# CleConor/rivulus

Measured on AMD Instinct MI355X. Metric: rows/sec filter+project, 1e9-row Int64, 10% selectivity, higher is better.
Workload: dtype int64

## Files before the change

rivulus_amd/csrc/core.hip:

```cpp
#include "launch.hpp"

using namespace rvh;
using namespace rvl;

namespace {
thread_local std::string g_last_error_text;
}
std::string &rvh::last_error() { return g_last_error_text; }

namespace rvl {

size_t elem_bytes(rv_dtype t, uint64_t n) {
    switch (t) {
        case RV_INT64:
        case RV_FLOAT64: return static_cast<size_t>(n) * 8;
        case RV_BOOLEAN: return static_cast<size_t>((n + 63) / 64) * 8;
        default: return 0;
    }
}
size_t bitmap_words_bytes(uint64_t n) { return static_cast<size_t>((n + 63) / 64) * 8; }

DevBufRef pool_alloc(rv_ctx *ctx, size_t bytes) {
    auto b = std::make_shared<DevBuf>();
    size_t got = 0;
// ... 73 lines not shown
    for (size_t i = 0; i < ctx->ctrl_free.size(); ++i)
        if (ctx->ctrl_free[i].bytes >= need) {
            c = ctx->ctrl_free[i];
            ctx->ctrl_free.erase(ctx->ctrl_free.begin() + static_cast<long>(i));
            break;
        }
    if (!c.dev) {
        if (!ctx->ctrl_free.empty()) {
            c = ctx->ctrl_free.back();
            ctx->ctrl_free.pop_back();
            RV_HIP(hipStreamSynchronize(ctx->stream));
            RV_HIP(hipFree(c.dev));
            c.dev = nullptr;
        } else {
            RV_HIP(hipHostMalloc(&c.host, kCtrlBytes, hipHostMallocDefault));
            RV_HIP(hipEventCreateWithFlags(&c.ev, hipEventDisableTiming));
        }
        c.bytes = std::max(need + need / 2, static_cast<size_t>(1) << 16);
        RV_HIP(hipMalloc(&c.dev, c.bytes));
    }
    RV_HIP(hipMemsetAsync(c.dev, 0, (zeroed + 15) & ~size_t(15), ctx->stream));
    c.clean = 0;
    c.dirty = zeroed;
    return c;
}
void release_launch_ctrl(rv_ctx *ctx, const rv_ctx::LaunchCtrl &c) { ctx->ctrl_free.push_back(c); }
int block_to_zero(rv_ctx *ctx, const rv_ctx::LaunchCtrl &like) {
    constexpr size_t kMost = size_t(64) << 20;
    for (size_t i = 0; i < ctx->ctrl_free.size(); ++i)
        if (ctx->ctrl_free[i].clean == 0 && ctx->ctrl_free[i].dirty > 0 && ctx->ctrl_free[i].dirty <= kMost) return static_cast<int>(i);
    bool any_clean = false;
    for (auto &f : ctx->ctrl_free) any_clean = any_clean || f.clean > 0;
    if (any_clean || ctx->ctrl_free.size() >= 3 || like.bytes > kMost) return -1;
    rv_ctx::LaunchCtrl c;
    if (hipHostMalloc(&c.host, kCtrlBytes, hipHostMallocDefault) != hipSuccess || hipEventCreateWithFlags(&c.ev, hipEventDisableTiming) != hipSuccess ||
        hipMalloc(&c.dev, like.bytes) != hipSuccess) {
        (void)hipGetLastError();
        if (c.host) (void)hipHostFree(c.host);
        if (c.ev) (void)hipEventDestroy(c.ev);
        return -1;
    }
    c.bytes = like.bytes;
    c.dirty = like.dirty;
    ctx->ctrl_free.push_back(c);
    return static_cast<int>(ctx->ctrl_free.size()) - 1;
}

rvk::DevCol dev_view(const rv_dcolumn *c) {
    rvk::DevCol d{};
    d.values = c->values ? c->values->ptr : nullptr;
// ... 86 lines not shown
    return count;
}

rv_status rv_ctx_create(int device, rv_ctx **out) {
    return guarded([&] {
        require(out != nullptr, RV_ERR_INVALID_ARG, "rv_ctx_create: out is NULL");
        int count = 0;
        hipError_t e = hipGetDeviceCount(&count);
        if (e != hipSuccess || count == 0) {
            (void)hipGetLastError();
            throw Error(RV_ERR_DEVICE, "no HIP device available: the MI355X backend has no CPU fallback");
        }
        require(device >= 0 && device < count, RV_ERR_INVALID_ARG, fmt("device %d out of range (%d present)", device, count));
        auto ctx = std::make_unique<rv_ctx>();
        ctx->device = device;
        RV_HIP(hipSetDevice(device));
        RV_HIP(hipGetDeviceProperties(&ctx->props, device));
        require(std::string(ctx->props.gcnArchName).rfind("gfx950", 0) == 0, RV_ERR_DEVICE,
                fmt("device %d is %s; this library carries gfx950 (MI355X) code objects only", device, ctx->props.gcnArchName));
        RV_HIP(hipStreamCreateWithFlags(&ctx->stream, hipStreamNonBlocking));
        RV_HIP(hipEventCreate(&ctx->ev0));
        RV_HIP(hipEventCreate(&ctx->ev1));
        RV_HIP(hipEventCreate(&ctx->evk0));
        RV_HIP(hipEventCreate(&ctx->evk1));
        RV_HIP(hipHostMalloc(&ctx->h_ctrl, kCtrlBytes, hipHostMallocDefault));
        RV_HIP(hipMalloc(&ctx->d_stripes, kStripeBytes));
        RV_HIP(hipMemset(ctx->d_stripes, 0, kStripeBytes));
        ctx->pool = std::make_shared<Pool>(device);
        if (const char *env = getenv("RV_OPTIONS")) {
            std::string all(env);
// ... 91 lines not shown
        else if (k == "stamp") ctx->opt_stamp = value;
        else if (k == "debug") ctx->opt_debug = value;
        else if (k == "depth") ctx->opt_depth = value;
        else if (k == "roomy") ctx->opt_roomy = value;
        else if (k == "direct") ctx->opt_direct = value;
        else if (k == "direct_r") ctx->opt_direct_r = value;
        else if (k == "sample") ctx->opt_sample = value;
        else if (k == "skew") ctx->opt_skew = value;
        else if (k == "segments") ctx->opt_segments = value;
        else if (k == "str_tiles_from") ctx->opt_str_tiles_from = value;
        else if (k == "groups_by_ranges") ctx->opt_groups_by_ranges = value;
        else if (k == "bool_cap") ctx->opt_bool_cap = value;
        else if (k == "speculative_batches") ctx->opt_speculative_batches = value;
        else if (k == "direct_waves") ctx->opt_direct_waves = value;
        else if (k == "spin_limit") ctx->opt_spin_limit = value;
        else if (k == "agg_grid") ctx->opt_agg_grid = value;
        else if (k == "bools_in_pass") ctx->opt_bools_in_pass = value;
        else if (k == "narrow_codes") {
            require(value >= -1 && value <= 2, RV_ERR_INVALID_ARG, "narrow_codes: 0 (auto), -1 (never), 1 (at the first whole scan, never packed) or 2 (at the first whole scan, packed where the rule allows)");
            ctx->opt_narrow_codes = value;
        }
        else if (k == "inject_failure") ctx->opt_inject_failure = value;
        else if (k == "csv_slow_cap") {
            require(value >= 0 && value < (int64_t(1) << 31), RV_ERR_INVALID_ARG, "csv_slow_cap must be in [0, 2^31)");
            ctx->opt_csv_slow_cap = value;
        }
        else if (k == "join_hash_bits") {
            require(value >= 0 && value < 64, RV_ERR_INVALID_ARG, "join_hash_bits must be in [0, 64)");
            ctx->opt_join_hash_bits = value;
        }
// ... 68 lines not shown
        else if (k == "csv_slow_cells") *value = static_cast<int64_t>(ctx->csv_slow_cells);
        else if (k == "csv_slow_reparses") *value = static_cast<int64_t>(ctx->csv_slow_reparses);
        else if (k == "inject_failure") *value = ctx->opt_inject_failure;
        else if (k == "join_hash_bits") *value = ctx->opt_join_hash_bits;
        else if (k == "string_hash_bits") *value = ctx->opt_string_hash_bits;
        else if (k == "agg_hash_bits") *value = ctx->opt_agg_hash_bits;
        else if (k == "agg_max_groups") *value = ctx->opt_agg_max_groups;
        else if (k == "sort_engine") *value = ctx->opt_sort_engine;
        else if (k == "sort_last_passes") *value = static_cast<int64_t>(ctx->sort_last_passes);
        else if (k == "top_k_select_from_rows") *value = ctx->opt_top_k_select_from_rows;
        else if (k == "top_k_refine_divisor") *value = ctx->opt_top_k_refine_divisor;
        else if (k == "top_k_last_passes") *value = static_cast<int64_t>(ctx->top_k_last_passes);
        else if (k == "top_k_last_candidates") *value = static_cast<int64_t>(ctx->top_k_last_candidates);
        else if (k == "out_sizing") *value = ctx->opt_out_sizing;
        else if (k == "overflow_reruns") *value = static_cast<int64_t>(ctx->overflow_reruns);
        else if (k == "batch_counts_in_pass") *value = static_cast<int64_t>(ctx->batch_counts_in_pass);
        else if (k == "fused_rows_scanned") *value = static_cast<int64_t>(ctx->fused_rows_scanned);
        else if (k == "last_redo_ppm") *value = static_cast<int64_t>(ctx->last_redo_fraction * 1e6);
        else if (k == "last_selectivity_ppm") *value = ctx->last_selectivity < 0 ? -1 : static_cast<int64_t>(ctx->last_selectivity * 1e6);
        else throw Error(RV_ERR_INVALID_ARG, "unknown option '" + k + "'");
    });
}

rv_status rv_ctx_kernel_stats(rv_ctx *ctx, double *total_ms, uint64_t *launches, int reset) {
    return guarded([&] {
        require(ctx != nullptr, RV_ERR_INVALID_ARG, "ctx is NULL");
        if (total_ms) *total_ms = ctx->kernel_ms;
        if (launches) *launches = ctx->kernel_launches;
        if (reset) {
            ctx->kernel_ms = 0.0;
// ... 29 lines not shown
```

rivulus_amd/csrc/fused_kernel.hpp:

```cpp
#pragma once

#include "lookback.hpp"
#include "narrow_sides.hpp"
#include "scan_frontend.hpp"
#include "tile_addr.hpp"

namespace rvk {

struct FusedParams {
    ScanInputs in;
    BitStream xs[kMaxBitStreams];
    uint64_t *out_values[kMaxValueCols];
    uint64_t *out_validity[kMaxValueCols];
    unsigned long long *out_valid_pop;
    uint64_t *out_selection;
    uint64_t *state;
    uint32_t *ticket;
    unsigned long long *out_count;
    uint32_t *err;
    uint32_t *overflow;
    uint64_t out_capacity;
    uint32_t *redo_count;
    unsigned long long *redo;
    unsigned long long *stamps;
    uint32_t ntiles;
    uint32_t cap_rows;
    int32_t nxs;
    int32_t debug;
    int32_t depth;
    uint32_t spin_limit;
    uint32_t out_bias;
    uint32_t *wave_counts;
    rv_u32x4 *zero_ptr;
    uint64_t zero_n16;
    unsigned long long *batch_counts;
    uint64_t nbatch_counts;
    uint64_t *wave_offsets;
    NarrowView narrow;
};

static_assert(kMaxTerms >= 4, "term slots 1 to 3 carry a one-term launch's code interval and tile constants");
__host__ __device__ inline void put_tile_walk(ScanInputs &in, const rvtile::TileWalk &w) {
    in.terms[2].lit = static_cast<int64_t>(w.view_byte0);
    in.terms[2].packed = w.tile_bytes;
    in.terms[2].pad = w.wave_bytes;
    in.terms[3].lit = static_cast<int64_t>(w.bytes);
    in.terms[3].packed = w.first_ragged_tile;
    in.terms[3].pad = w.ragged_rows;
}
__host__ __device__ inline rvtile::TileWalk get_tile_walk(const ScanInputs &in) {
    rvtile::TileWalk w{};
    w.view_byte0 = static_cast<uint64_t>(in.terms[2].lit);
    w.tile_bytes = in.terms[2].packed;
    w.wave_bytes = in.terms[2].pad;
// ... 859 lines not shown
            atomicAdd(&d[1], st_scatter);
            atomicAdd(&d[2], st_look);
            atomicAdd(&d[3], st_waitB);
            atomicAdd(&d[4], st_flush);
            atomicAdd(&d[5], st_tiles);
            if (wave == 1) {
                atomicAdd(&d[6], st_wait);
                atomicAdd(&d[7], st_stage);
            }
        }
    }

    if (__syncthreads_or(n_redo != 0)) {
        if (lane == 0 && n_redo) atomicAdd(s_redo, n_redo);
        __syncthreads();
        if (threadIdx.x == 0) atomicAdd(p.redo_count, *s_redo);
    }

    if constexpr (kValidity || kXs) {
        __syncthreads();
        const uint32_t *s_pop = reinterpret_cast<const uint32_t *>(smem + 24);
        if (threadIdx.x < kMaxValueCols + kMaxBitStreams && s_pop[threadIdx.x])
            atomicAdd(&p.out_valid_pop[threadIdx.x], static_cast<unsigned long long>(s_pop[threadIdx.x]));
    }
}

#undef RV_TILE_PARAM
#undef RV_TILE_WRITES

constexpr int kRedoWaves = 4;
template <int NCOLS, int RR>
// ... 125 lines not shown
```

rivulus_amd/csrc/fused_launch.hip:

```cpp
#include "fused_rule.hpp"
#include "launch.hpp"
#include "narrow_sides.hpp"
#include "narrow_term.hpp"
#include "tile_addr.hpp"

#include <cmath>

using namespace rvh;
using namespace rvl;

namespace rvk {
const FusedEntry *fused_entries(size_t *n) {
    static const std::vector<FusedEntry> all = [] {
        std::vector<FusedEntry> v;
        for (auto *source : {fused_entries_lean1, fused_entries_valid1, fused_entries_multi, fused_entries_bool, fused_entries_full, fused_entries_expr,
                             fused_entries_roomy, fused_entries_narrow}) {
            size_t k = 0;
            const FusedEntry *t = source(&k);
            v.insert(v.end(), t, t + k);
        }
        return v;
    }();
    *n = all.size();
    return all.data();
// ... 108 lines not shown
        mix(ex->negate_result ? 3 : 2);
        for (size_t t = 0; t < ex->negate.size(); ++t) mix(static_cast<uint64_t>(ex->negate[t]) | (static_cast<uint64_t>(ex->group_end[t]) << 8));
    }
    return signature;
}

static void launch_redo(rv_ctx *ctx, FusedLaunch &L) {
    const int rr = L.nvals ? rvk::redo_rows_per_lane(L.nvals, L.range_rows) : 4;
    const rvk::RedoFn redo = rvk::redo_kernel(L.nvals, rr);
    require(redo != nullptr && L.nranges > 0, RV_ERR_INTERNAL, "no redo kernel variant");
    const size_t redo_lds = rvk::kLdsHeader + static_cast<size_t>(rvk::kRedoWaves) * (std::max(L.nvals, 1) + rvk::kMaxBitStreams) * 64 * rr;
    const uint64_t want = (L.nranges + rvk::kRedoWaves - 1) / rvk::kRedoWaves;
    const uint32_t rgrid = static_cast<uint32_t>(std::min<uint64_t>(want, static_cast<uint64_t>(ctx->props.multiProcessorCount) * 8));
    hipLaunchKernelGGL(redo, dim3(rgrid), dim3(rvk::kRedoWaves * 64), redo_lds, ctx->stream, L.p, L.range_rows, L.nranges);
    RV_HIP(hipGetLastError());
}

struct Bound {
    const rv_dcolumn *const *cols;
    rvk::ScanInputs *in;
    std::vector<int> value_slot, bool_slot;
    std::vector<char> never_null;
    int nvals = 0, nbools = 0, npred = 0;

    int add_value(const rv_dcolumn *col) {
        require(nvals < rvk::kMaxValueCols, RV_ERR_UNSUPPORTED, "too many 8-byte columns for one pass");
        in->cols[nvals] = dev_view(col);
        return nvals++;
    }
    int value_of(uint32_t c) {
// ... 350 lines not shown
}

static void launch_pass(rv_ctx *ctx, FusedLaunch &L, const LaunchChoice &c, int nvals, rv_dcolumn **sel_out, BatchReq *req, RangeOffsets *ranges,
                        double seen) {
    rvk::FusedParams &p = L.p;
    if (c.make_selection) make_selection(ctx, L, sel_out);
    p.ntiles = c.ntiles;
    p.cap_rows = c.cap;
    p.depth = static_cast<int32_t>(c.stages) - 1;

    L.range_rows = 64u * static_cast<uint32_t>(c.r);
    L.nranges = c.direct ? 0 : static_cast<uint64_t>(p.ntiles) * c.waves;
    L.ctrl = acquire_launch_ctrl(ctx, p.ntiles, L.nranges);
    Ctrl *ctrl = static_cast<Ctrl *>(L.ctrl.dev);
    p.state = reinterpret_cast<uint64_t *>(static_cast<unsigned char *>(L.ctrl.dev) + kCtrlBytes);
    p.ticket = &ctrl->ticket;
    p.err = &ctrl->err;
    p.out_count = &ctrl->out_count;
    p.out_valid_pop = ctrl->valid_pop;
    p.stamps = ctrl->stamps;
    p.debug = static_cast<int32_t>(ctx->opt_debug);
    p.spin_limit = ctx->opt_spin_limit > 0 ? static_cast<uint32_t>(ctx->opt_spin_limit) : rvk::kSpinLimit;
    p.redo_count = &ctrl->redo_count;
    p.redo = L.nranges ? reinterpret_cast<unsigned long long *>(static_cast<unsigned char *>(L.ctrl.dev) + kCtrlBytes + static_cast<size_t>(p.ntiles) * 8) : nullptr;

    const void *fn = reinterpret_cast<const void *>(c.fn);
    enable_lds(ctx, fn, c.lds);
    if (c.narrow) {
        const bool packed = c.narrow->layout == rvn::Layout::kPacked;
        p.narrow.codes = c.narrow->codes->ptr;
        p.narrow.bytes = packed ? std::min<uint64_t>(c.narrow->codes->bytes, rvn::packed_bytes(c.narrow->count)) : c.narrow->codes->bytes;
        p.narrow.base = c.narrow->base;
        require(p.in.nterms == 1, RV_ERR_INTERNAL, "narrow pass: one term");
// ... 7 lines not shown
        p.in.terms[1].pad = (packed && interval) ? static_cast<uint32_t>(rvn::classify_sides(ct.lo, ct.span, c.narrow->range)) : 0u;
        L.plain = {c.staged->fn_plain, c.lds_plain, static_cast<int32_t>(c.stages_plain) - 1};
        ctx->narrow_passes += 1;
    }
    auto occ = ctx->occupancy.find({fn, c.lds});
    if (occ == ctx->occupancy.end()) {
        int q = 0;
        RV_HIP(hipOccupancyMaxActiveBlocksPerMultiprocessor(&q, fn, c.waves * 64, c.lds));
        occ = ctx->occupancy.emplace(std::make_pair(fn, c.lds), std::max(1, q)).first;
    }
    int per_cu = occ->second;
    if (ctx->opt_wgs_per_cu > 0) per_cu = static_cast<int>(ctx->opt_wgs_per_cu);
    uint64_t workers = std::min<uint64_t>(p.ntiles, static_cast<uint64_t>(ctx->props.multiProcessorCount) * per_cu - 1);
    if (ctx->opt_grid_limit > 0 && !c.direct) workers = std::min<uint64_t>(workers, static_cast<uint64_t>(ctx->opt_grid_limit));
    const uint32_t grid = 1 + static_cast<uint32_t>(workers);
    p.overflow = &ctrl->overflow;
    if (ranges) {
        ranges->range_rows = 64u * static_cast<uint32_t>(c.r);
        ranges->out_capacity = p.out_capacity;
        ranges->expected_selectivity = seen;
        if (4096u % ranges->range_rows == 0) {
            ranges->offsets = pool_alloc(ctx, static_cast<size_t>(p.ntiles) * c.waves * 8 + 16);
            p.wave_offsets = static_cast<uint64_t *>(ranges->offsets->ptr);
        }
    }
    if (counts_in_pass(req, c.r)) {
        if (req->chunk_rows == 64u * static_cast<uint64_t>(c.r)) {
            p.batch_counts = req->counts;
            p.nbatch_counts = req->nb;
            req->counted = true;
            ctx->batch_counts_in_pass += 1;
// ... 39 lines not shown
    p.zero_n16 = 0;
    L.redo_queued = L.nranges && (c.redo_expected > 0.0 || L.place_edge) && (c.stage_row_bytes || p.nxs);
    if (L.redo_queued) launch_redo(ctx, L);
    if (L.timed) RV_HIP(hipEventRecord(L.ctrl.tk1, ctx->stream));
    if (p.wave_counts) {
        const uint64_t per_batch = req->chunk_rows / (64u * static_cast<uint64_t>(c.r)), nwaves = static_cast<uint64_t>(p.ntiles) * c.waves;
        const uint64_t threads = per_batch < 32 ? req->nb : (per_batch < 4096 ? req->nb * 64 : req->nb * 256);
        const dim3 cgrid(static_cast<uint32_t>(std::max<uint64_t>(1, std::min<uint64_t>((threads + 255) / 256, static_cast<uint64_t>(ctx->props.multiProcessorCount) * 8))));
        hipLaunchKernelGGL(rvk::batch_counts_from_waves, cgrid, dim3(256), 0, ctx->stream, static_cast<const uint32_t *>(p.wave_counts), nwaves, per_batch, req->nb, req->counts);
        RV_HIP(hipGetLastError());
        req->counted = true;
        ctx->batch_counts_in_pass += 1;
        p.wave_counts = nullptr;
    }
    p.batch_counts = nullptr;
    RV_HIP(hipMemcpyAsync(L.ctrl.host, L.ctrl.dev, kCtrlBytes, hipMemcpyDeviceToHost, ctx->stream));
    RV_HIP(hipEventRecord(L.ctrl.ev, ctx->stream));
    L.launched = true;
}

void fused_begin(rv_ctx *ctx, const rv_dcolumn *const *cols, uint32_t ncols, const rv_term *terms,
                 uint32_t nterms, rv_null_policy policy, const uint32_t *proj, uint32_t nproj,
                 rv_dcolumn **out, rv_dcolumn **sel_out, FusedLaunch &L, const ExprInfo *ex, BatchReq *req,
                 RangeOffsets *ranges) {
    rvk::FusedParams &p = L.p;
    p = rvk::FusedParams{};
    Bound b = bind_inputs(cols, ncols, terms, nterms, policy, ex, p.in);
    const uint64_t n = p.in.n;
    L.signature = predicate_signature(cols, ncols, terms, nterms, policy, ex);
    double seen = L.place ? L.place_selectivity : ctx->seen_selectivity(L.signature);
    bool sampled_now = false;
// ... 44 lines not shown
}

uint64_t fused_finish(rv_ctx *ctx, FusedLaunch &L) {
    if (!L.launched) return 0;
    rvk::FusedParams &p = L.p;
    std::vector<OutCol> &outs = L.outs;
    struct Release {
        rv_ctx *ctx;
        FusedLaunch &L;
        ~Release() {
            L.wave_counts.reset();
            release_launch_ctrl(ctx, L.ctrl);
            L.launched = false;
        }
    } release{ctx, L};
    RV_HIP(hipEventSynchronize(L.ctrl.ev));
    L.wave_counts.reset();
    const Ctrl *h = static_cast<const Ctrl *>(L.ctrl.host);
    if (L.timed) {
        float ms = 0.f;
        RV_HIP(hipEventElapsedTime(&ms, L.ctrl.tk0, L.ctrl.tk1));
        ctx->kernel_ms += ms;
        ctx->kernel_launches += 1;
    }
    require(h->err == 0, RV_ERR_DEVICE, "fused kernel: look-back spin limit reached (device fault or lost workgroup)");
    ctx->last_selectivity = L.n ? static_cast<double>(h->out_count) / static_cast<double>(L.n) : 0.0;
    ctx->last_rows_out = h->out_count, ctx->last_rows_in = L.n;
    if (!L.place) ctx->remember_selectivity(L.signature, ctx->last_selectivity);
    bool rerun = false;
    if (L.place && (h->overflow || h->out_count > p.out_capacity)) {
        L.overflowed = true;
        throw SegmentOverflow{};
    }
    if (h->overflow || h->out_count > p.out_capacity) {
        rerun = true;
        const uint64_t exact = h->out_count;
        alloc_outputs(ctx, L, exact);
        const size_t zeroed = kCtrlBytes + (static_cast<size_t>(p.ntiles) + L.nranges) * 8;
        RV_HIP(hipMemsetAsync(L.ctrl.dev, 0, (zeroed + 15) & ~size_t(15), ctx->stream));
        if (L.plain.fn) {
            enable_lds(ctx, reinterpret_cast<const void *>(L.plain.fn), L.plain.lds);
            p.depth = L.plain.depth;
        }
        hipLaunchKernelGGL(L.plain.fn ? L.plain.fn : L.fn, dim3(L.grid), dim3(L.block), L.plain.fn ? L.plain.lds : L.lds, ctx->stream, p);
        RV_HIP(hipGetLastError());
        RV_HIP(hipMemcpyAsync(L.ctrl.host, L.ctrl.dev, kCtrlBytes, hipMemcpyDeviceToHost, ctx->stream));
        RV_HIP(hipStreamSynchronize(ctx->stream));
        require(h->err == 0 && h->overflow == 0 && h->out_count == exact, RV_ERR_INTERNAL, "re-run after an output overflow disagrees with the first pass");
        ctx->overflow_reruns += 1;
    }
    ctx->last_redo_fraction = L.nranges ? static_cast<double>(h->redo_count) / static_cast<double>(L.nranges) : 0.0;
    if (L.nranges && !L.place) {
        if (rv_ctx::SeenPredicate *q = ctx->seen_entry(L.signature)) {
            q->redo_fraction = ctx->last_redo_fraction, q->redo_at = ctx->last_selectivity;
            q->redo_ratio = L.range_rows ? static_cast<double>(p.cap_rows) / L.range_rows : 1.0;
        }
    }
    if (h->redo_count > 0 && (L.stage_row_bytes || p.nxs) && !(L.redo_queued && !rerun)) {
        if (L.timed) RV_HIP(hipEventRecord(ctx->evk0, ctx->stream));
        launch_redo(ctx, L);
        if (L.timed) RV_HIP(hipEventRecord(ctx->evk1, ctx->stream));
        RV_HIP(hipMemcpyAsync(L.ctrl.host, L.ctrl.dev, kCtrlBytes, hipMemcpyDeviceToHost, ctx->stream));
        RV_HIP(hipStreamSynchronize(ctx->stream));
        if (L.timed) {
            float ms = 0.f;
            RV_HIP(hipEventElapsedTime(&ms, ctx->evk0, ctx->evk1));
            ctx->kernel_ms += ms;
        }
        require(h->overflow == 0, RV_ERR_INTERNAL, "redo kernel: outputs too small after the pass fitted them");
    }
    const uint64_t rows = h->out_count;
    if (ctx->opt_debug & 4)
        fprintf(stderr, "[scan] tiles %llu | scanner polls %llu, tiles scanned %llu, empty polls %llu | fallback look-backs %llu\n",
                static_cast<unsigned long long>(p.ntiles), h->stamps[28], h->stamps[29], h->stamps[30], h->stamps[31]);
    if ((ctx->opt_debug & 4) && L.nranges == 0)
        fprintf(stderr, "[scan] direct kernel: tiles whose predecessor's prefix was not there at the top of the iteration: looked again once %llu, twice %llu, three times %llu, four %llu\n",
                h->stamps[16], h->stamps[17], h->stamps[18], h->stamps[19]);
    if (L.direct_stamp) {
        const double t = static_cast<double>(p.ntiles);
        const unsigned long long *q = h->stamps;
        fprintf(stderr, "[stamp direct] cycles/tile (s_memtime, wave 1): load wait %.0f | predicate+count %.0f | barrier 1 %.0f | publish..offset (wave 0: %.0f) %.0f | barrier 2 %.0f | stores %.0f | barrier 3 %.0f | moves+load issue %.0f\n",
                q[0] / t, q[1] / t, q[2] / t, q[8] / t, q[3] / t, q[4] / t, q[5] / t, q[6] / t, q[7] / t);
    }
    if ((L.need & rvk::FF_STAMP) && ctx->opt_stamp) {
        std::memcpy(ctx->last_stamps, h->stamps, sizeof(h->stamps));
        for (int w = 0; w < 2; ++w) {
// ... 223 lines not shown
```

rivulus_amd/csrc/launch.hpp:

```cpp
#pragma once

#include <algorithm>
#include <array>
#include <chrono>
#include <functional>
#include <thread>

#include "aux_kernels.hpp"
#include "fused_table.hpp"
#include "string_kernels.hpp"
#include "runtime.hpp"
#include "thresholds.hpp"

namespace rvk {
struct RangesCompact;
}

namespace rvl {
using namespace rvh;

constexpr size_t kCtrlBytes = 512;
constexpr size_t kStripeBytes = static_cast<size_t>(rvk::kStripeSlots) * rvk::kStripeSlotWords * 8;
struct Ctrl {
    uint32_t ticket;
    uint32_t err;
    unsigned long long out_count;
    unsigned long long valid_pop[8];
    unsigned long long pops[3];
    unsigned long long pad0[3];
    rvk::AggPartial agg;
    unsigned long long stamps[32];
    uint32_t redo_count;
    uint32_t overflow;
};

static_assert(sizeof(Ctrl) <= kCtrlBytes, "ctrl block");
static_assert(offsetof(Ctrl, agg) == 128, "ctrl layout");

size_t elem_bytes(rv_dtype t, uint64_t n);
size_t bitmap_words_bytes(uint64_t n);
inline size_t zeroed_bitmap_bytes(uint64_t n) { return (bitmap_words_bytes(n) + 8 + 255) & ~static_cast<size_t>(255); }
DevBufRef pool_alloc(rv_ctx *ctx, size_t bytes);
void set_device(rv_ctx *ctx);
void maybe_injected_failure(rv_ctx *ctx);
Ctrl *prepare_ctrl(rv_ctx *ctx, size_t ntiles);
unsigned long long *striped(rv_ctx *ctx, const unsigned long long *ctrl_word);
const Ctrl *fetch_ctrl(rv_ctx *ctx);
rv_ctx::LaunchCtrl acquire_launch_ctrl(rv_ctx *ctx, size_t ntiles, size_t nranges = 0);
void release_launch_ctrl(rv_ctx *ctx, const rv_ctx::LaunchCtrl &c);
int block_to_zero(rv_ctx *ctx, const rv_ctx::LaunchCtrl &like);
rvk::DevCol dev_view(const rv_dcolumn *c);
bool is_value_type(rv_dtype t);
// ... 27 lines not shown
    DevBufRef offsets;
    uint32_t range_rows = 0;
    uint64_t out_capacity = 0;
    double expected_selectivity = -1.0;
};

struct FusedLaunch {
    rvk::FusedParams p{};
    std::vector<OutCol> outs;
    rv_ctx::LaunchCtrl ctrl;
    int need = 0, nvals = 0;
    size_t stage_row_bytes = 0;
    uint32_t range_rows = 0;
    uint64_t nranges = 0;
    bool launched = false;
    DevBufRef wave_counts;
    bool redo_queued = false;
    bool timed = false;
    bool direct_stamp = false;
    void (*fn)(const rvk::FusedParams) = nullptr;
    uint32_t grid = 0, block = 0;
    size_t lds = 0;
    uint64_t n = 0;
    uint64_t signature = 0;
    const std::vector<DevBufRef> *place = nullptr;
    uint64_t place_base = 0, place_capacity = 0;
    double place_selectivity = -1.0;
    bool place_edge = false;
    bool overflowed = false;
    uint32_t out_bias = 0;
// ... 5 lines not shown
        size_t lds = 0;
        int32_t depth = 2;
    } plain;
};
struct SegmentOverflow {};

using AfterLaunch = std::function<void(const rv_dcolumn *sel)>;

uint64_t output_capacity(rv_ctx *ctx, uint64_t n, double expected);
double expected_selectivity(rv_ctx *ctx, const rv_dcolumn *const *cols, uint32_t ncols, const rv_term *terms, uint32_t nterms, rv_null_policy policy, const ExprInfo *ex);
uint64_t predicate_signature(const rv_dcolumn *const *cols, uint32_t ncols, const rv_term *terms, uint32_t nterms, rv_null_policy policy, const ExprInfo *ex);
void fused_begin(rv_ctx *ctx, const rv_dcolumn *const *cols, uint32_t ncols, const rv_term *terms, uint32_t nterms, rv_null_policy policy,
                 const uint32_t *proj, uint32_t nproj, rv_dcolumn **out, rv_dcolumn **sel_out, FusedLaunch &L, const ExprInfo *ex = nullptr,
                 BatchReq *req = nullptr, RangeOffsets *ranges = nullptr);
uint64_t fused_finish(rv_ctx *ctx, FusedLaunch &L);
void abandon_launch(rv_ctx *ctx, FusedLaunch &L);
uint64_t run_fused_pass(rv_ctx *ctx, const rv_dcolumn *const *cols, uint32_t ncols, const rv_term *terms, uint32_t nterms, rv_null_policy policy,
                        const uint32_t *proj, uint32_t nproj, rv_dcolumn **out, rv_dcolumn **sel_out, const ExprInfo *ex = nullptr, BatchReq *req = nullptr,
                        const AfterLaunch *after_launch = nullptr, RangeOffsets *ranges = nullptr);
bool run_segmented_pass(rv_ctx *ctx, const rv_dcolumn *const *cols, uint32_t ncols, const rv_term *terms, uint32_t nterms, rv_null_policy policy,
                        const uint32_t *proj, uint32_t nproj, rv_dcolumn **out, const ExprInfo *ex, uint64_t *rows_out);

struct StrSelLaunch {
    std::unique_ptr<rv_dcolumn> col;
    const rv_dcolumn *src = nullptr;
    DevBufRef lengths, starts, block_sums, groups;
    uint64_t cap_rows = 0;
    Ctrl *ctrl = nullptr;
    int slot = 0;
    bool queued = false;
// ... 83 lines not shown
```

rivulus_amd/csrc/lookback.hpp:

```cpp
#pragma once

#include "device_common.hpp"

namespace rvk {

constexpr uint64_t kStAgg = 1ull << 62;
constexpr uint64_t kStPfx = 2ull << 62;
constexpr uint64_t kStVal = (1ull << 62) - 1;
constexpr uint32_t kSpinLimit = 1u << 22;

__device__ __forceinline__ uint64_t ld_state(const uint64_t *p) {
    return __hip_atomic_load(p, __ATOMIC_RELAXED, __HIP_MEMORY_SCOPE_AGENT);
}
__device__ __forceinline__ void st_state(uint64_t *p, uint64_t v) {
    __hip_atomic_store(p, v, __ATOMIC_RELAXED, __HIP_MEMORY_SCOPE_AGENT);
}

constexpr int kLookK = 8;

__device__ __forceinline__ void publish_aggregate(uint64_t *state, uint32_t tile, uint64_t aggregate, uint32_t first) {
    st_state(&state[tile], tile == 0 ? (kStPfx | (aggregate + first)) : (kStAgg | aggregate));
}

__device__ __forceinline__ void lookback_issue(const uint64_t *state, int64_t base, int lane, uint64_t (&s)[kLookK]) {
// ... 28 lines not shown
            if (im & below) {
                ready = false;
            } else {
                const uint64_t take = below | nearest;
                contrib += ((take >> lane) & 1) ? (s[k] & kStVal) : 0;
                found = pm != 0;
            }
        }
        if (ready) {
            excl += wave_sum64(contrib);
            ++windows;
            if (found) break;
            base -= 64 * kLookK;
        } else {
            if (++spins > spin_limit) {
                if (lane == 0) atomicExch(err, 1u);
                break;
            }
            __builtin_amdgcn_s_sleep(2);
        }
        lookback_issue(state, base, lane, s);
        ++polls;
    }
    if (poll_stats && lane == 0) {
        atomicAdd(&poll_stats[0], static_cast<unsigned long long>(polls));
        atomicAdd(&poll_stats[1], static_cast<unsigned long long>(windows));
    }
    excl = uniform64(excl);
    if (lane == 0) st_state(&state[tile], kStPfx | ((excl + aggregate) & kStVal));
    return excl;
}
// ... 56 lines not shown
```

rivulus_amd/csrc/query.hip:

```cpp
#include "launch.hpp"
#include "ranges_kernel.hpp"

using namespace rvh;
using namespace rvl;

namespace rvl {
struct MaskWindow {
    rv_ctx::LaunchCtrl ctrl;
    bool launched = false;
    std::unique_ptr<rv_dcolumn> sel;
    DevBufRef counts;
    RangeOffsets ranges;
    std::vector<const rv_dcolumn *> src;
    uint64_t n = 0, assumed = 0, signature = 0;
};
enum class MaskTotal { kWait, kInContext, kInWindow };

static bool mask_shape(const rv_ctx *ctx, const rv_dcolumn *const *cols, uint32_t ncols, const rv_term *terms, uint32_t nterms, rv_null_policy policy,
                       bool expr, uint64_t chunk_rows) {
    const uint64_t n = ncols ? cols[0]->length : 0;
    return ctx->opt_groups_by_ranges >= 0 && !expr && nterms == 1 && terms[0].op == RV_IS_TRUE && policy == RV_NULL_DROPS && terms[0].column < ncols &&
           cols[terms[0].column]->dtype == RV_BOOLEAN && (n >= rvt::kRangesFromRows || (ctx->opt_groups_by_ranges == 1 && n > 0)) && chunk_rows % 1024 == 0;
}
static uint64_t assumed_rows(uint64_t n, double known) {
// ... 1028 lines not shown
    mask_compact(ctx, w, cap, outs);
    ctx->last_kernel = fmt("compact_ranges_kernel<%d>", static_cast<int>(std::min<size_t>(rvk::kRangesMaxCols, w.src.size())));
}
static void mask_window_begin(rv_ctx *ctx, const rv_dcolumn *const *cols, const rv_predicate *pred, const uint32_t *proj, uint32_t nproj, BatchReq &req,
                              double known, uint64_t signature, MaskWindow &w, rv_dcolumn **outs) {
    const rv_dcolumn *mask = cols[pred->terms[0].column];
    w.signature = signature;
    w.assumed = assumed_rows(mask->length, known);
    mask_select_begin(ctx, mask, &req, MaskTotal::kInWindow, w);
    for (uint32_t j = 0; j < nproj; ++j) {
        outs[j] = new_value_column(ctx, cols[proj[j]]->dtype, w.assumed).release();
        w.src.push_back(cols[proj[j]]);
    }
    mask_window_compact(ctx, w, w.assumed, outs);
    RV_HIP(hipMemcpyAsync(w.ctrl.host, w.ctrl.dev, kCtrlBytes, hipMemcpyDeviceToHost, ctx->stream));
    RV_HIP(hipEventRecord(w.ctrl.ev, ctx->stream));
}
static uint64_t mask_window_finish(rv_ctx *ctx, MaskWindow &w, rv_dcolumn **outs, uint32_t nproj) {
    RV_HIP(hipEventSynchronize(w.ctrl.ev));
    const uint64_t rows = static_cast<const Ctrl *>(w.ctrl.host)->pops[0];
    release_launch_ctrl(ctx, w.ctrl);
    w.launched = false;
    if (rows > w.assumed) {
        for (uint32_t j = 0; j < nproj; ++j) outs[j]->values = pool_alloc(ctx, std::max<size_t>(elem_bytes(outs[j]->dtype, rows), 8));
        mask_window_compact(ctx, w, rows, outs);
        RV_HIP(hipStreamSynchronize(ctx->stream));
        ctx->overflow_reruns += 1;
    }
    for (uint32_t j = 0; j < nproj; ++j) outs[j]->length = rows;
    ctx->remember_selectivity(w.signature, w.n ? static_cast<double>(rows) / static_cast<double>(w.n) : 0.0);
    ctx->last_selectivity = w.n ? static_cast<double>(rows) / static_cast<double>(w.n) : 0.0;
    ctx->last_rows_out = rows, ctx->last_rows_in = w.n;
    return rows;
}
// ... 215 lines not shown
```

rivulus_amd/csrc/runtime.hpp:

```cpp
#pragma once

#include <hip/hip_runtime.h>

#include <atomic>
#include <cstdarg>
#include <cstdio>
#include <cstring>
#include <map>
#include <memory>
#include <mutex>
#include <stdexcept>
#include <string>
#include <vector>

#include "../../include/rivulus_gpu.h"
#include "narrow_rule.hpp"

namespace rvh {

struct Error : std::runtime_error {
    rv_status status;
    Error(rv_status s, const std::string &m) : std::runtime_error(m), status(s) {}
};

// ... 201 lines not shown
    uint64_t samples_taken = 0;
    uint64_t last_rows_out = 0, last_rows_in = 0;
    int64_t opt_speculative_batches = 0;
    uint64_t speculative_batch_passes = 0;
    int64_t opt_str_tiles_from = 0;
    int64_t opt_bool_cap = 0;
    int64_t opt_groups_by_ranges = 0;
    int64_t opt_sample = 0;
    int64_t opt_segments = 0;
    uint64_t segmented_passes = 0;
    uint64_t segment_fallbacks = 0;
    int64_t opt_skew = 0;
    uint64_t fused_rows_scanned = 0;
    uint64_t batch_counts_in_pass = 0;
    uint64_t overflow_reruns = 0;
    int64_t opt_inject_failure = 0;
    bool undrained = false;
    int64_t opt_join_hash_bits = 0;
    int64_t opt_string_hash_bits = 0;
    int64_t opt_agg_hash_bits = 0;
    int64_t opt_agg_max_groups = 0;
    int64_t opt_sort_engine = 0;
    uint64_t sort_last_passes = 0;
    int64_t opt_top_k_select_from_rows = 0;
    int64_t opt_top_k_refine_divisor = 0;
    uint64_t top_k_last_passes = 0;
    uint64_t top_k_last_candidates = 0;
    int64_t opt_bools_in_pass = 0;
    int64_t opt_narrow_codes = 0;
    uint64_t narrow_builds = 0;
    uint64_t narrow_passes = 0;
    uint64_t narrow_bytes = 0;
    int64_t opt_csv_slow_cap = 0;
    uint64_t csv_slow_cells = 0;
    uint64_t csv_slow_reparses = 0;
    unsigned long long last_stamps[32] = {};
    std::map<std::pair<const void *, size_t>, int> occupancy;
    std::map<const void *, size_t> lds_enabled;
    struct LaunchCtrl {
        void *dev = nullptr;
        size_t bytes = 0;
        void *host = nullptr;
        hipEvent_t ev = nullptr;
        hipEvent_t tk0 = nullptr, tk1 = nullptr;
        size_t clean = 0, dirty = 0;
    };
    std::vector<LaunchCtrl> ctrl_free;
    void *h_stage = nullptr;
    size_t stage_bytes = 0;
    void *stage(size_t bytes) {
        if (bytes > stage_bytes) {
            if (h_stage) (void)hipHostFree(h_stage);
            h_stage = nullptr;
            stage_bytes = 0;
            const size_t want = std::max(bytes + bytes / 2, static_cast<size_t>(1) << 20);
            if (hipHostMalloc(&h_stage, want, hipHostMallocDefault) != hipSuccess) {
                (void)hipGetLastError();
// ... 8 lines not shown
```

rivulus_amd/csrc/thresholds.hpp:

```cpp
#pragma once
#include <cstdint>

namespace rvt {
constexpr uint64_t kSampleFromRows = uint64_t{1} << 25;
constexpr double kDirectFromOneColumn = 0.52;
constexpr double kDirectFromOneProjectedOfSeveral = 0.60;
constexpr double kDirectFromTwoProjected = 0.22;
constexpr double kDirectFromThreeProjected = 0.15;
constexpr double kDirectFromTwoProjectedNullable = 0.35;
constexpr double kDirectFromThreeProjectedNullable = 0.22;
constexpr double kDirectTallBelow = 0.62;
constexpr double kCrowdedMargin = 1.1, kCrowdedSigmas = 3.0;
constexpr double kRedoMsPerShare = 3.5, kDirectPenaltyAt0 = 0.9, kDirectPenaltySlope = 1.3, kDirectPenaltyFloor = 0.1;
constexpr double kRedoMemorySelectivityBand = 0.15, kRedoMemorySlotBand = 0.05;
constexpr uint64_t kOutSizingFromRows = uint64_t{1} << 25;
constexpr double kOutSizingFactor = 1.2, kOutSizingSlack = 0.02;
constexpr double kStretchSparseUpTo = 0.30, kStretchDenseFrom = 0.55, kStretchKnownBand = 0.05;
constexpr int kStretchLeastBlocks = 24, kStretchesMost = 4;
constexpr uint64_t kStretchFromRows = uint64_t{1} << 28;

constexpr uint64_t kNarrowAfterWholeScans = 2;
constexpr uint64_t kNarrowFromRows = uint64_t{1} << 25;

constexpr uint64_t kRangesFromRows = uint64_t{1} << 24;
constexpr double kDeferPlainUpTo = 0.25;
constexpr uint64_t kRangesSparseNum = 11, kRangesSparseDen = 20;
constexpr double kMaskPathPlainUpTo = 0.55;
constexpr double kMaskPathAssumeUpTo = 0.5;

constexpr uint32_t kSpeculateFromBatches = 4096;
constexpr uint32_t kWalkThreadsFromBatches = 16384;
constexpr uint32_t kWalkThreads = 8;

constexpr double kStrTilesFrom = 0.50;
// ... 21 lines not shown
```

Before: 2532 billion.

## Write fused-scan results straight to pinned host memory and spin-wait on completion

For simple launches with no stamps, bit streams or validity outputs, the kernel now writes err, out_count and overflow directly into mapped pinned host memory. This removes the device-to-host control-block copy after each pass. A redo flag tells the host when the full block must still be copied for redo_count. The host also polls the completion event for up to a configurable microsecond budget before falling back to a blocking sync, trading CPU spin for lower wake-up latency.

```diff
diff --git a/rivulus_amd/csrc/core.hip b/rivulus_amd/csrc/core.hip
--- a/rivulus_amd/csrc/core.hip
+++ b/rivulus_amd/csrc/core.hip
@@ -111,6 +111,7 @@
             c.dev = nullptr;
         } else {
             RV_HIP(hipHostMalloc(&c.host, kCtrlBytes, hipHostMallocDefault));
+            RV_HIP(hipHostGetDevicePointer(&c.host_dev, c.host, 0));
             RV_HIP(hipEventCreateWithFlags(&c.ev, hipEventDisableTiming));
         }
         c.bytes = std::max(need + need / 2, static_cast<size_t>(1) << 16);
@@ -130,7 +131,7 @@
     for (auto &f : ctx->ctrl_free) any_clean = any_clean || f.clean > 0;
     if (any_clean || ctx->ctrl_free.size() >= 3 || like.bytes > kMost) return -1;
     rv_ctx::LaunchCtrl c;
-    if (hipHostMalloc(&c.host, kCtrlBytes, hipHostMallocDefault) != hipSuccess || hipEventCreateWithFlags(&c.ev, hipEventDisableTiming) != hipSuccess ||
+    if (hipHostMalloc(&c.host, kCtrlBytes, hipHostMallocDefault) != hipSuccess || hipHostGetDevicePointer(&c.host_dev, c.host, 0) != hipSuccess || hipEventCreateWithFlags(&c.ev, hipEventDisableTiming) != hipSuccess ||
         hipMalloc(&c.dev, like.bytes) != hipSuccess) {
         (void)hipGetLastError();
         if (c.host) (void)hipHostFree(c.host);
@@ -247,6 +248,7 @@
         require(device >= 0 && device < count, RV_ERR_INVALID_ARG, fmt("device %d out of range (%d present)", device, count));
         auto ctx = std::make_unique<rv_ctx>();
         ctx->device = device;
+        ctx->opt_wait_spin_us = rvt::kWaitSpinUs;
         RV_HIP(hipSetDevice(device));
         RV_HIP(hipGetDeviceProperties(&ctx->props, device));
         require(std::string(ctx->props.gcnArchName).rfind("gfx950", 0) == 0, RV_ERR_DEVICE,
@@ -368,6 +370,10 @@
         else if (k == "speculative_batches") ctx->opt_speculative_batches = value;
         else if (k == "direct_waves") ctx->opt_direct_waves = value;
         else if (k == "spin_limit") ctx->opt_spin_limit = value;
+        else if (k == "wait_spin_us") {
+            require(value >= 0 && value <= 10000000, RV_ERR_INVALID_ARG, "wait_spin_us: 0 (the runtime's wait only) or a polling budget in microseconds, up to 10 s");
+            ctx->opt_wait_spin_us = value;
+        }
         else if (k == "agg_grid") ctx->opt_agg_grid = value;
         else if (k == "bools_in_pass") ctx->opt_bools_in_pass = value;
         else if (k == "narrow_codes") {
@@ -466,6 +472,9 @@
         else if (k == "top_k_last_candidates") *value = static_cast<int64_t>(ctx->top_k_last_candidates);
         else if (k == "out_sizing") *value = ctx->opt_out_sizing;
         else if (k == "overflow_reruns") *value = static_cast<int64_t>(ctx->overflow_reruns);
+        else if (k == "wait_spin_us") *value = ctx->opt_wait_spin_us;
+        else if (k == "results_on_host") *value = static_cast<int64_t>(ctx->results_on_host);
+        else if (k == "result_copies") *value = static_cast<int64_t>(ctx->result_copies);
         else if (k == "batch_counts_in_pass") *value = static_cast<int64_t>(ctx->batch_counts_in_pass);
         else if (k == "fused_rows_scanned") *value = static_cast<int64_t>(ctx->fused_rows_scanned);
         else if (k == "last_redo_ppm") *value = static_cast<int64_t>(ctx->last_redo_fraction * 1e6);
diff --git a/rivulus_amd/csrc/fused_kernel.hpp b/rivulus_amd/csrc/fused_kernel.hpp
--- a/rivulus_amd/csrc/fused_kernel.hpp
+++ b/rivulus_amd/csrc/fused_kernel.hpp
@@ -38,6 +38,11 @@
     uint64_t *wave_offsets;
     NarrowView narrow;
 };
+
+constexpr int kRedoFlagBytesPastCount = 96;
+__device__ inline uint32_t *redo_flag_of(unsigned long long *out_count) {
+    return reinterpret_cast<uint32_t *>(reinterpret_cast<unsigned char *>(out_count) + kRedoFlagBytesPastCount);
+}
 
 static_assert(kMaxTerms >= 4, "term slots 1 to 3 carry a one-term launch's code interval and tile constants");
 __host__ __device__ inline void put_tile_walk(ScanInputs &in, const rvtile::TileWalk &w) {
@@ -927,7 +932,10 @@
     if (__syncthreads_or(n_redo != 0)) {
         if (lane == 0 && n_redo) atomicAdd(s_redo, n_redo);
         __syncthreads();
-        if (threadIdx.x == 0) atomicAdd(p.redo_count, *s_redo);
+        if (threadIdx.x == 0) {
+            atomicAdd(p.redo_count, *s_redo);
+            *redo_flag_of(p.out_count) = 1u;
+        }
     }
 
     if constexpr (kValidity || kXs) {
diff --git a/rivulus_amd/csrc/fused_launch.hip b/rivulus_amd/csrc/fused_launch.hip
--- a/rivulus_amd/csrc/fused_launch.hip
+++ b/rivulus_amd/csrc/fused_launch.hip
@@ -2,6 +2,7 @@
 #include "launch.hpp"
 #include "narrow_sides.hpp"
 #include "narrow_term.hpp"
+#include "result_words.hpp"
 #include "tile_addr.hpp"
 
 #include <cmath>
@@ -146,6 +147,56 @@
     const uint32_t rgrid = static_cast<uint32_t>(std::min<uint64_t>(want, static_cast<uint64_t>(ctx->props.multiProcessorCount) * 8));
     hipLaunchKernelGGL(redo, dim3(rgrid), dim3(rvk::kRedoWaves * 64), redo_lds, ctx->stream, L.p, L.range_rows, L.nranges);
     RV_HIP(hipGetLastError());
+}
+
+constexpr rvw::Flags kResultFlags = {rvk::FF_STAMP, rvk::FF_XS, rvk::FF_OUTVALID};
+
+void wait_for_launch(rv_ctx *ctx, hipEvent_t ev) {
+    hipError_t last = hipSuccess;
+    const int failed = rvw::wait_bounded(
+        ctx->opt_wait_spin_us,
+        [&] {
+            last = hipEventQuery(ev);
+            if (last != hipErrorNotReady) return last == hipSuccess ? 0 : 2;
+            (void)hipGetLastError();
+            return 1;
+        },
+        [&] {
+            last = hipEventSynchronize(ev);
+            return last == hipSuccess ? 0 : 2;
+        },
+        [] { return static_cast<int64_t>(std::chrono::duration_cast<std::chrono::microseconds>(std::chrono::steady_clock::now().time_since_epoch()).count()); },
+        [] {
+#if defined(__x86_64__)
+            __builtin_ia32_pause();
+#else
+            std::this_thread::yield();
+#endif
+        });
+    if (failed) RV_HIP(last);
+}
+
+static void reset_host_words(FusedLaunch &L) {
+    Ctrl *h = static_cast<Ctrl *>(L.ctrl.host);
+    h->err = 0, h->out_count = 0, h->overflow = 0, h->redo_flag = 0, h->redo_count = 0;
+}
+static void queue_result_copy(rv_ctx *ctx, FusedLaunch &L) {
+    RV_HIP(hipMemcpyAsync(L.ctrl.host, L.ctrl.dev, kCtrlBytes, hipMemcpyDeviceToHost, ctx->stream));
+    ctx->result_copies += 1;
+}
+static void fetch_redo_count(rv_ctx *ctx, FusedLaunch &L) {
+    Ctrl *h = static_cast<Ctrl *>(L.ctrl.host);
+    if (!h->redo_flag && !h->err) return;
+    const Ctrl own = *h;
+    queue_result_copy(ctx, L);
+    RV_HIP(hipStreamSynchronize(ctx->stream));
+    h->err = own.err, h->out_count = own.out_count, h->overflow = own.overflow, h->redo_flag = own.redo_flag;
+    L.copied = true;
+}
+static void fetch_results(rv_ctx *ctx, FusedLaunch &L, bool redo_count) {
+    if (!L.on_host) queue_result_copy(ctx, L);
+    RV_HIP(hipStreamSynchronize(ctx->stream));
+    if (L.on_host && redo_count) fetch_redo_count(ctx, L);
 }
 
 struct Bound {
@@ -526,9 +577,15 @@
     L.ctrl = acquire_launch_ctrl(ctx, p.ntiles, L.nranges);
     Ctrl *ctrl = static_cast<Ctrl *>(L.ctrl.dev);
     p.state = reinterpret_cast<uint64_t *>(static_cast<unsigned char *>(L.ctrl.dev) + kCtrlBytes);
+    int nv_out = 0;
+    for (int s = 0; s < nvals; ++s) nv_out += p.out_validity[s] != nullptr;
+    L.on_host = rvw::results_on_host(kResultFlags, {c.flags, nv_out, p.nxs, ctx->opt_debug, ctx->opt_stamp != 0});
+    L.copied = false;
+    Ctrl *results = L.on_host ? static_cast<Ctrl *>(L.ctrl.host_dev) : ctrl;
+    if (L.on_host) reset_host_words(L);
     p.ticket = &ctrl->ticket;
-    p.err = &ctrl->err;
-    p.out_count = &ctrl->out_count;
+    p.err = &results->err;
+    p.out_count = &results->out_count;
     p.out_valid_pop = ctrl->valid_pop;
     p.stamps = ctrl->stamps;
     p.debug = static_cast<int32_t>(ctx->opt_debug);
@@ -566,7 +623,7 @@
     uint64_t workers = std::min<uint64_t>(p.ntiles, static_cast<uint64_t>(ctx->props.multiProcessorCount) * per_cu - 1);
     if (ctx->opt_grid_limit > 0 && !c.direct) workers = std::min<uint64_t>(workers, static_cast<uint64_t>(ctx->opt_grid_limit));
     const uint32_t grid = 1 + static_cast<uint32_t>(workers);
-    p.overflow = &ctrl->overflow;
+    p.overflow = &results->overflow;
     if (ranges) {
         ranges->range_rows = 64u * static_cast<uint32_t>(c.r);
         ranges->out_capacity = p.out_capacity;
@@ -636,7 +693,7 @@
         p.wave_counts = nullptr;
     }
     p.batch_counts = nullptr;
-    RV_HIP(hipMemcpyAsync(L.ctrl.host, L.ctrl.dev, kCtrlBytes, hipMemcpyDeviceToHost, ctx->stream));
+    if (!L.on_host) queue_result_copy(ctx, L);
     RV_HIP(hipEventRecord(L.ctrl.ev, ctx->stream));
     L.launched = true;
 }
@@ -711,9 +768,10 @@
             L.launched = false;
         }
     } release{ctx, L};
-    RV_HIP(hipEventSynchronize(L.ctrl.ev));
+    wait_for_launch(ctx, L.ctrl.ev);
     L.wave_counts.reset();
     const Ctrl *h = static_cast<const Ctrl *>(L.ctrl.host);
+    if (L.on_host) fetch_redo_count(ctx, L);
     if (L.timed) {
         float ms = 0.f;
         RV_HIP(hipEventElapsedTime(&ms, L.ctrl.tk0, L.ctrl.tk1));
@@ -735,14 +793,14 @@
         alloc_outputs(ctx, L, exact);
         const size_t zeroed = kCtrlBytes + (static_cast<size_t>(p.ntiles) + L.nranges) * 8;
         RV_HIP(hipMemsetAsync(L.ctrl.dev, 0, (zeroed + 15) & ~size_t(15), ctx->stream));
+        if (L.on_host) reset_host_words(L);
         if (L.plain.fn) {
             enable_lds(ctx, reinterpret_cast<const void *>(L.plain.fn), L.plain.lds);
             p.depth = L.plain.depth;
         }
         hipLaunchKernelGGL(L.plain.fn ? L.plain.fn : L.fn, dim3(L.grid), dim3(L.block), L.plain.fn ? L.plain.lds : L.lds, ctx->stream, p);
         RV_HIP(hipGetLastError());
-        RV_HIP(hipMemcpyAsync(L.ctrl.host, L.ctrl.dev, kCtrlBytes, hipMemcpyDeviceToHost, ctx->stream));
-        RV_HIP(hipStreamSynchronize(ctx->stream));
+        fetch_results(ctx, L, true);
         require(h->err == 0 && h->overflow == 0 && h->out_count == exact, RV_ERR_INTERNAL, "re-run after an output overflow disagrees with the first pass");
         ctx->overflow_reruns += 1;
     }
@@ -757,8 +815,7 @@
         if (L.timed) RV_HIP(hipEventRecord(ctx->evk0, ctx->stream));
         launch_redo(ctx, L);
         if (L.timed) RV_HIP(hipEventRecord(ctx->evk1, ctx->stream));
-        RV_HIP(hipMemcpyAsync(L.ctrl.host, L.ctrl.dev, kCtrlBytes, hipMemcpyDeviceToHost, ctx->stream));
-        RV_HIP(hipStreamSynchronize(ctx->stream));
+        fetch_results(ctx, L, false);
         if (L.timed) {
             float ms = 0.f;
             RV_HIP(hipEventElapsedTime(&ms, ctx->evk0, ctx->evk1));
@@ -767,6 +824,7 @@
         require(h->overflow == 0, RV_ERR_INTERNAL, "redo kernel: outputs too small after the pass fitted them");
     }
     const uint64_t rows = h->out_count;
+    if (L.on_host && !L.copied) ctx->results_on_host += 1;
     if (ctx->opt_debug & 4)
         fprintf(stderr, "[scan] tiles %llu | scanner polls %llu, tiles scanned %llu, empty polls %llu | fallback look-backs %llu\n",
                 static_cast<unsigned long long>(p.ntiles), h->stamps[28], h->stamps[29], h->stamps[30], h->stamps[31]);
diff --git a/rivulus_amd/csrc/launch.hpp b/rivulus_amd/csrc/launch.hpp
--- a/rivulus_amd/csrc/launch.hpp
+++ b/rivulus_amd/csrc/launch.hpp
@@ -27,7 +27,9 @@
     unsigned long long out_count;
     unsigned long long valid_pop[8];
     unsigned long long pops[3];
-    unsigned long long pad0[3];
+    uint32_t redo_flag;
+    uint32_t pad1;
+    unsigned long long pad0[2];
     rvk::AggPartial agg;
     unsigned long long stamps[32];
     uint32_t redo_count;
@@ -36,6 +38,7 @@
 
 static_assert(sizeof(Ctrl) <= kCtrlBytes, "ctrl block");
 static_assert(offsetof(Ctrl, agg) == 128, "ctrl layout");
+static_assert(offsetof(Ctrl, redo_flag) == offsetof(Ctrl, out_count) + rvk::kRedoFlagBytesPastCount, "the kernels find redo_flag from out_count");
 
 size_t elem_bytes(rv_dtype t, uint64_t n);
 size_t bitmap_words_bytes(uint64_t n);
@@ -93,6 +96,8 @@
     uint32_t range_rows = 0;
     uint64_t nranges = 0;
     bool launched = false;
+    bool on_host = false;
+    bool copied = false;
     DevBufRef wave_counts;
     bool redo_queued = false;
     bool timed = false;
@@ -128,6 +133,7 @@
                  const uint32_t *proj, uint32_t nproj, rv_dcolumn **out, rv_dcolumn **sel_out, FusedLaunch &L, const ExprInfo *ex = nullptr,
                  BatchReq *req = nullptr, RangeOffsets *ranges = nullptr);
 uint64_t fused_finish(rv_ctx *ctx, FusedLaunch &L);
+void wait_for_launch(rv_ctx *ctx, hipEvent_t ev);
 void abandon_launch(rv_ctx *ctx, FusedLaunch &L);
 uint64_t run_fused_pass(rv_ctx *ctx, const rv_dcolumn *const *cols, uint32_t ncols, const rv_term *terms, uint32_t nterms, rv_null_policy policy,
                         const uint32_t *proj, uint32_t nproj, rv_dcolumn **out, rv_dcolumn **sel_out, const ExprInfo *ex = nullptr, BatchReq *req = nullptr,
diff --git a/rivulus_amd/csrc/lookback.hpp b/rivulus_amd/csrc/lookback.hpp
--- a/rivulus_amd/csrc/lookback.hpp
+++ b/rivulus_amd/csrc/lookback.hpp
@@ -66,7 +66,7 @@
             base -= 64 * kLookK;
         } else {
             if (++spins > spin_limit) {
-                if (lane == 0) atomicExch(err, 1u);
+                if (lane == 0) *err = 1u;
                 break;
             }
             __builtin_amdgcn_s_sleep(2);
diff --git a/rivulus_amd/csrc/query.hip b/rivulus_amd/csrc/query.hip
--- a/rivulus_amd/csrc/query.hip
+++ b/rivulus_amd/csrc/query.hip
@@ -1066,10 +1066,11 @@
     }
     mask_window_compact(ctx, w, w.assumed, outs);
     RV_HIP(hipMemcpyAsync(w.ctrl.host, w.ctrl.dev, kCtrlBytes, hipMemcpyDeviceToHost, ctx->stream));
+    ctx->result_copies += 1;
     RV_HIP(hipEventRecord(w.ctrl.ev, ctx->stream));
 }
 static uint64_t mask_window_finish(rv_ctx *ctx, MaskWindow &w, rv_dcolumn **outs, uint32_t nproj) {
-    RV_HIP(hipEventSynchronize(w.ctrl.ev));
+    wait_for_launch(ctx, w.ctrl.ev);
     const uint64_t rows = static_cast<const Ctrl *>(w.ctrl.host)->pops[0];
     release_launch_ctrl(ctx, w.ctrl);
     w.launched = false;
diff --git a/rivulus_amd/csrc/result_words.hpp b/rivulus_amd/csrc/result_words.hpp
--- /dev/null
+++ b/rivulus_amd/csrc/result_words.hpp
@@ -0,0 +1,42 @@
+#pragma once
+
+#include <stdint.h>
+
+namespace rvw {
+
+struct Flags {
+    int stamp;
+    int xs;
+    int outvalid;
+};
+
+struct Launch {
+    int flags;
+    int validity_outputs;
+    int bit_streams;
+    int64_t debug;
+    bool stamp;
+};
+
+inline bool results_on_host(const Flags &f, const Launch &l) {
+    if (l.flags & (f.stamp | f.xs | f.outvalid)) return false;
+    if (l.validity_outputs > 0 || l.bit_streams > 0) return false;
+    return l.debug == 0 && !l.stamp;
+}
+
+template <class Query, class Block, class Now, class Pause>
+int wait_bounded(int64_t budget_us, Query query, Block block, Now now, Pause pause) {
+    int q = query();
+    if (q != 1) return q;
+    if (budget_us > 0) {
+        const int64_t t0 = now();
+        while (now() - t0 < budget_us) {
+            pause();
+            q = query();
+            if (q != 1) return q;
+        }
+    }
+    return block();
+}
+
+}
diff --git a/rivulus_amd/csrc/runtime.hpp b/rivulus_amd/csrc/runtime.hpp
--- a/rivulus_amd/csrc/runtime.hpp
+++ b/rivulus_amd/csrc/runtime.hpp
@@ -239,6 +239,9 @@
     uint64_t fused_rows_scanned = 0;
     uint64_t batch_counts_in_pass = 0;
     uint64_t overflow_reruns = 0;
+    uint64_t results_on_host = 0;
+    uint64_t result_copies = 0;
+    int64_t opt_wait_spin_us = 0;
     int64_t opt_inject_failure = 0;
     bool undrained = false;
     int64_t opt_join_hash_bits = 0;
@@ -266,6 +269,7 @@
         void *dev = nullptr;
         size_t bytes = 0;
         void *host = nullptr;
+        void *host_dev = nullptr;
         hipEvent_t ev = nullptr;
         hipEvent_t tk0 = nullptr, tk1 = nullptr;
         size_t clean = 0, dirty = 0;
diff --git a/rivulus_amd/csrc/thresholds.hpp b/rivulus_amd/csrc/thresholds.hpp
--- a/rivulus_amd/csrc/thresholds.hpp
+++ b/rivulus_amd/csrc/thresholds.hpp
@@ -18,6 +18,8 @@
 constexpr double kStretchSparseUpTo = 0.30, kStretchDenseFrom = 0.55, kStretchKnownBand = 0.05;
 constexpr int kStretchLeastBlocks = 24, kStretchesMost = 4;
 constexpr uint64_t kStretchFromRows = uint64_t{1} << 28;
+
+constexpr int64_t kWaitSpinUs = 1000;
 
 constexpr uint64_t kNarrowAfterWholeScans = 2;
 constexpr uint64_t kNarrowFromRows = uint64_t{1} << 25;
```

Result: no change. 2523 billion, median of 2 (-0.3%).
